# facebookresearch/robust_cvd

Measured on NVIDIA H100. Metric: flow_residual_constraints_per_sec_per_gn_iteration, higher is better.
Workload: dtype f64

## Files before the change

### robust_cvd_b200/csrc/rcvd_linalg.cuh

```cuda
#pragma once
#include "rcvd_device.cuh"

namespace rcvd {

constexpr int kPotrfThreads = 256;

__global__ void __launch_bounds__(kPotrfThreads) k_potrf_panel(double* __restrict__ Lb, double* __restrict__ invT,
                                                                const int* __restrict__ frames, int npad, int jb, int* __restrict__ fail) {
  __shared__ double D[16][17];
  __shared__ double Di[16][17];
  const int frame = frames[blockIdx.x];
  double* A = Lb + (size_t)frame * npad * npad;
  double* iT = invT + (size_t)frame * npad * 16;
  const int tid = threadIdx.x;
  const int j0 = jb * 16;
  {
    const int r = tid >> 4, cc = tid & 15;
    D[r][cc] = (cc <= r) ? A[(size_t)(j0 + r) * npad + j0 + cc] : 0.0;
  }
  __syncthreads();
  if (tid < 32) {
    const int i = tid;
    for (int j = 0; j < 16; ++j) {
      if (i == j) {
        double d = D[j][j];
        for (int q = 0; q < j; ++q) d -= D[j][q] * D[j][q];
        if (!(d > 0.0) || !isfinite(d)) { *fail = 1; d = 1.0; }
        D[j][j] = sqrt(d);
      }
      __syncwarp();
      if (i > j && i < 16) {
        double s = D[i][j];
        for (int q = 0; q < j; ++q) s -= D[i][q] * D[j][q];
        D[i][j] = s / D[j][j];
      }
      __syncwarp();
    }
    if (i < 16) {
      const int cidx = i;
      double xcol[16];
#pragma unroll
      for (int r = 0; r < 16; ++r) {
        double s = (r == cidx) ? 1.0 : 0.0;
#pragma unroll
        for (int q = 0; q < 16; ++q) if (q < r) s -= D[r][q] * xcol[q];
        xcol[r] = (r < cidx) ? 0.0 : s / D[r][r];
      }
#pragma unroll
      for (int r = 0; r < 16; ++r) Di[r][cidx] = xcol[r];
    }
  }
  __syncthreads();
  {
    const int r = tid >> 4, cc = tid & 15;
    A[(size_t)(j0 + r) * npad + j0 + cc] = D[r][cc];
    iT[(size_t)jb * 256 + r * 16 + cc] = Di[r][cc];
  }
  const int below = npad - (j0 + 16);
  for (int rr = tid; rr < below; rr += kPotrfThreads) {
    double a[16], xo[16];
    double* row = A + (size_t)(j0 + 16 + rr) * npad + j0;
#pragma unroll
    for (int q = 0; q < 16; ++q) a[q] = row[q];
#pragma unroll
    for (int cc = 0; cc < 16; ++cc) {
      double s = 0.0;
#pragma unroll
      for (int q = 0; q < 16; ++q) if (q <= cc) s += a[q] * Di[cc][q];
      xo[cc] = s;
    }
#pragma unroll
    for (int q = 0; q < 16; ++q) row[q] = xo[q];
  }
}

constexpr int kPotrfSmemThreads = 512;
constexpr int kTileSz = 256;
__host__ __device__ inline size_t potrf_smem_bytes(int npad) { const int nt = npad / 16; return (size_t)(nt * (nt + 1) / 2 + 1) * kTileSz * sizeof(double); }
__device__ __forceinline__ int swz(int r, int k) { return r * 16 + (k ^ ((r & 3) << 2)); }
__device__ __forceinline__ void cp_async16_fwd(void* smem, const void* gmem) {
  const unsigned sa = (unsigned)__cvta_generic_to_shared(smem);
  asm volatile("cp.async.cg.shared.global [%0], [%1], 16;" ::"r"(sa), "l"(gmem) : "memory");
}
__device__ __forceinline__ void dmma_8x8x4_fwd(double& c0, double& c1, double a, double b) {
  asm volatile("mma.sync.aligned.m8n8k4.row.col.f64.f64.f64.f64 {%0,%1}, {%2}, {%3}, {%0,%1};"
               : "+d"(c0), "+d"(c1) : "d"(a), "d"(b));
}

__device__ __forceinline__ void tile_mma_nt(const double* __restrict__ At, const double* __restrict__ Bt, double acc[2][2][2], int g, int t) {
#pragma unroll
  for (int k4 = 0; k4 < 4; ++k4) {
    double af[2], bf[2];
#pragma unroll
    for (int i = 0; i < 2; ++i) { af[i] = At[swz(i * 8 + g, k4 * 4 + t)]; bf[i] = Bt[swz(i * 8 + g, k4 * 4 + t)]; }
#pragma unroll
    for (int i = 0; i < 2; ++i)
#pragma unroll
      for (int j = 0; j < 2; ++j) dmma_8x8x4_fwd(acc[i][j][0], acc[i][j][1], af[i], bf[j]);
  }
}

__device__ __forceinline__ void warp_chol16(double* __restrict__ D, double* __restrict__ pinv, int lane, int* __restrict__ fail) {
  const int i = lane & 15;
  double a[16];
#pragma unroll
  for (int c = 0; c < 16; ++c) a[c] = (c <= i) ? D[swz(i, c)] : 0.0;
#pragma unroll
  for (int j = 0; j < 16; ++j) {
    double d = __shfl_sync(0xffffffffu, a[j], j);
    if (!(d > 0.0) || !isfinite(d)) { if (lane == 0) *fail = 1; d = 1.0; }
    const double pi = rsqrt(d);
    const double lij = (i == j) ? d * pi : a[j] * pi;
    if (i >= j) a[j] = lij;
    if (lane == 0) pinv[j] = pi;
#pragma unroll
    for (int c = 0; c < 16; ++c) {
      if (c > j) {
        const double lcj = __shfl_sync(0xffffffffu, a[j], c);
        if (i >= c) a[c] -= lij * lcj;
      }
    }
  }
  if (lane < 16) {
#pragma unroll
    for (int c = 0; c < 16; ++c) D[swz(i, c)] = a[c];
  }
}

#ifdef RCVD_POTRF_PHASES
__device__ long long g_potrf_phase[16];
#define POTRF_PHASE(n) do { if (threadIdx.x == 0 && blockIdx.x == 0) { const long long now_ = clock64(); g_potrf_phase[n] += now_ - last_; last_ = now_; } } while (0)
#define CHOL_PHASE(n) do { if (threadIdx.x == 0 && blockIdx.x == 0) { const long long now_ = clock64(); g_potrf_phase[n] += now_ - cl_; cl_ = now_; } } while (0)
#else
#define CHOL_PHASE(n) do { } while (0)
#define POTRF_PHASE(n) do { } while (0)
#endif

__device__ __forceinline__ void warp_chol16_blocked(double* __restrict__ D, double* __restrict__ pinv, int lane, int* __restrict__ fail) {
  const int g = lane >> 2, t = lane & 3;
  double c[3][2];
  const int ui[3] = {0, 1, 1}, uj[3] = {0, 0, 1};
#pragma unroll
  for (int u = 0; u < 3; ++u) { const double2 v = *reinterpret_cast<const double2*>(&D[swz(8 * ui[u] + g, 8 * uj[u] + 2 * t)]); c[u][0] = v.x; c[u][1] = v.y; }
  bool bad = false;
#ifdef RCVD_POTRF_PHASES
  long long cl_ = clock64();
#endif
#pragma unroll
  for (int b = 0; b < 4; ++b) {
    const int k0 = 4 * b;
    if (b > 0) {
#pragma unroll
      for (int u = 0; u < 3; ++u) if (8 * uj[u] + 2 * t >= k0) *reinterpret_cast<double2*>(&D[swz(8 * ui[u] + g, 8 * uj[u] + 2 * t)]) = make_double2(c[u][0], c[u][1]);
    }
    __syncwarp();
    double a00 = D[swz(k0, k0)], a10 = D[swz(k0 + 1, k0)], a11 = D[swz(k0 + 1, k0 + 1)], a20 = D[swz(k0 + 2, k0)], a21 = D[swz(k0 + 2, k0 + 1)],
           a22 = D[swz(k0 + 2, k0 + 2)], a30 = D[swz(k0 + 3, k0)], a31 = D[swz(k0 + 3, k0 + 1)], a32 = D[swz(k0 + 3, k0 + 2)], a33 = D[swz(k0 + 3, k0 + 3)];
    CHOL_PHASE(8);
    double t01 = a10 * a10;
    double det01 = fma(a00, a11, -t01);
    if (!(a00 > 0.0) || !isfinite(a00)) { bad = true; a00 = 1.0; det01 = 1.0; }
    if (!(det01 > 0.0) || !isfinite(det01)) { bad = true; det01 = a00; }
    const double p0 = rsqrt(a00), r01 = rsqrt(det01);
    const double sq0 = a00 * p0;
    const double p1 = r01 * sq0;
    const double l11 = det01 * r01 * p0;
    const double l10 = a10 * p0, l20 = a20 * p0, l30 = a30 * p0;
    const double l21 = (a21 - l20 * l10) * p1, l31 = (a31 - l30 * l10) * p1;
    double b22 = fma(-l21, l21, fma(-l20, l20, a22)), b33 = fma(-l31, l31, fma(-l30, l30, a33));
    const double b32 = fma(-l31, l21, fma(-l30, l20, a32));
    double det23 = fma(b22, b33, -(b32 * b32));
    if (!(b22 > 0.0) || !isfinite(b22)) { bad = true; b22 = 1.0; det23 = 1.0; }
    if (!(det23 > 0.0) || !isfinite(det23)) { bad = true; det23 = b22; }
    const double p2 = rsqrt(b22), r23 = rsqrt(det23);
    const double sq2 = b22 * p2;
    const double p3 = r23 * sq2;
    const double l33 = det23 * r23 * p2;
    const double l32 = b32 * p2;
    CHOL_PHASE(9);
    const int r = lane & 15;
    const bool below = lane < 16 && r >= k0 + 4;
    double x0 = D[swz(r, k0)] * p0;
    double x1 = (D[swz(r, k0 + 1)] - x0 * l10) * p1;
    double x2 = (D[swz(r, k0 + 2)] - x0 * l20 - x1 * l21) * p2;
    double x3 = (D[swz(r, k0 + 3)] - x0 * l30 - x1 * l31 - x2 * l32) * p3;
    if (below) { D[swz(r, k0)] = x0; D[swz(r, k0 + 1)] = x1; D[swz(r, k0 + 2)] = x2; D[swz(r, k0 + 3)] = x3; }
    __syncwarp();
    CHOL_PHASE(10);
    if (lane == 0) {
      *reinterpret_cast<double2*>(&D[swz(k0, k0)]) = make_double2(sq0, 0.0);         *reinterpret_cast<double2*>(&D[swz(k0, k0 + 2)]) = make_double2(0.0, 0.0);
      *reinterpret_cast<double2*>(&D[swz(k0 + 1, k0)]) = make_double2(l10, l11);     *reinterpret_cast<double2*>(&D[swz(k0 + 1, k0 + 2)]) = make_double2(0.0, 0.0);
      *reinterpret_cast<double2*>(&D[swz(k0 + 2, k0)]) = make_double2(l20, l21);          *reinterpret_cast<double2*>(&D[swz(k0 + 2, k0 + 2)]) = make_double2(sq2, 0.0);
      *reinterpret_cast<double2*>(&D[swz(k0 + 3, k0)]) = make_double2(l30, l31);          *reinterpret_cast<double2*>(&D[swz(k0 + 3, k0 + 2)]) = make_double2(l32, l33);
      *reinterpret_cast<double2*>(&pinv[k0]) = make_double2(p0, p1);                      *reinterpret_cast<double2*>(&pinv[k0 + 2]) = make_double2(p2, p3);
    }
    if (b < 3) {
      double pa[2];
#pragma unroll
      for (int i = 0; i < 2; ++i) { const int r = 8 * i + g; pa[i] = r >= k0 + 4 ? D[swz(r, k0 + t)] : 0.0; }
#pragma unroll
      for (int u = 0; u < 3; ++u) dmma_8x8x4_fwd(c[u][0], c[u][1], -pa[ui[u]], pa[uj[u]]);
    }
    CHOL_PHASE(11);
  }
  if (bad && lane == 0) *fail = 1;
}


__global__ void __launch_bounds__(kPotrfSmemThreads) k_potrf_smem(double* __restrict__ Lb, double* __restrict__ invT,
                                                                   const int* __restrict__ frames, int npad, int* __restrict__ fail, int chain_warp) {
  extern __shared__ __align__(16) double tiles[];
  const int frame = frames[blockIdx.x];
  double* A = Lb + (size_t)frame * npad * npad;
  double* iT = invT + (size_t)frame * npad * 16;
  const int nt = npad / 16, ntl = nt * (nt + 1) / 2;
  double* pinv = tiles + (size_t)ntl * kTileSz;
  const int tid = threadIdx.x, warp = tid >> 5, lane = tid & 31, nw = kPotrfSmemThreads / 32;
  const int g = lane >> 2, t = lane & 3;
#ifdef RCVD_POTRF_PHASES
  long long last_ = clock64();
#endif
  for (int idx = tid; idx < ntl * 128; idx += kPotrfSmemThreads) {
    const int tl = idx >> 7, e = idx & 127, r = e >> 3, c = (e & 7) * 2;
    int ti = (int)((sqrtf(8.f * tl + 1.f) - 1.f) * 0.5f);
    while ((ti + 1) * (ti + 2) / 2 <= tl) ++ti;
    while (ti * (ti + 1) / 2 > tl) --ti;
    const int tj = tl - ti * (ti + 1) / 2;
    cp_async16_fwd(&tiles[(size_t)tl * kTileSz + swz(r, c)], &A[(size_t)(ti * 16 + r) * npad + tj * 16 + c]);
  }
  asm volatile("cp.async.commit_group;" ::: "memory");
  asm volatile("cp.async.wait_group 0;" ::: "memory");
  __syncthreads();
  POTRF_PHASE(0);
  if (warp == 0) { if (chain_warp & 2) warp_chol16_blocked(tiles, pinv, lane, fail); else warp_chol16(tiles, pinv, lane, fail); }
  __syncthreads();
  POTRF_PHASE(1);
  for (int jb = 0; jb < nt; ++jb) {
    const double* D = tiles + (size_t)(jb * (jb + 1) / 2 + jb) * kTileSz;
    const double* pv = pinv + jb * 16;
    const int rows = (nt - jb - 1) * 16;
    const bool chain = (chain_warp & 1) != 0;
    int prow = -1;
    const int nwork = nw - 1, widx = warp - 1;
    if (chain) { if (warp == 0) { if (lane < 16 && rows > 0) prow = lane; } else if (widx * 32 + lane < rows - 16) prow = 16 + widx * 32 + lane; }
    else if (tid < rows) prow = tid;
    if (chain && warp != 0) asm volatile("bar.sync 2, %0;" ::"n"(kPotrfSmemThreads) : "memory");
    if (prow >= 0) {
      const int ti = jb + 1 + (prow >> 4), r = prow & 15;
      double* Tt = tiles + (size_t)(ti * (ti + 1) / 2 + jb) * kTileSz;
      double a[16];
#pragma unroll
      for (int q = 0; q < 16; q += 2) { const double2 v = *reinterpret_cast<const double2*>(&Tt[swz(r, q)]); a[q] = v.x; a[q + 1] = v.y; }
#pragma unroll
      for (int q = 0; q < 16; q += 2) {
        const double2 pq = *reinterpret_cast<const double2*>(&pv[q]);
        const double2 dq = *reinterpret_cast<const double2*>(&D[swz(q + 1, q)]);
        a[q] *= pq.x;
        a[q + 1] = (a[q + 1] - a[q] * dq.x) * pq.y;
#pragma unroll
        for (int c = 0; c < 16; ++c) if (c > q + 1) { const double2 l = *reinterpret_cast<const double2*>(&D[swz(c, q)]); a[c] -= a[q] * l.x; a[c] -= a[q + 1] * l.y; }
      }
#pragma unroll
      for (int q = 0; q < 16; q += 2) *reinterpret_cast<double2*>(&Tt[swz(r, q)]) = make_double2(a[q], a[q + 1]);
    } else if (warp == nw - 1 && lane < 16) {
      const int cidx = lane;
      double xcol[16];
#pragma unroll
      for (int r = 0; r < 16; ++r) xcol[r] = (r == cidx) ? 1.0 : 0.0;
#pragma unroll
      for (int q = 0; q < 16; q += 2) {
        const double2 pq = *reinterpret_cast<const double2*>(&pv[q]);
        const double2 dq = *reinterpret_cast<const double2*>(&D[swz(q + 1, q)]);
        xcol[q] *= pq.x;
        xcol[q + 1] = (xcol[q + 1] - xcol[q] * dq.x) * pq.y;
#pragma unroll
        for (int r = 0; r < 16; ++r) if (r > q + 1) { const double2 l = *reinterpret_cast<const double2*>(&D[swz(r, q)]); xcol[r] -= l.x * xcol[q]; xcol[r] -= l.y * xcol[q + 1]; }
      }
#pragma unroll
      for (int r = 0; r < 16; ++r) iT[(size_t)jb * 256 + r * 16 + cidx] = xcol[r];
    }
    POTRF_PHASE(2);
    if (!chain) __syncthreads();
    else if (warp != 0) asm volatile("bar.sync 3, %0;" ::"n"(kPotrfSmemThreads - 32) : "memory");
    POTRF_PHASE(3);
    const int m = nt - jb - 1, ntr = m * (m + 1) / 2;
    auto upd_tile = [&](int gi, int gj) -> double* {
      const double* Xi = tiles + (size_t)(gi * (gi + 1) / 2 + jb) * kTileSz;
      const double* Xj = tiles + (size_t)(gj * (gj + 1) / 2 + jb) * kTileSz;
      double* Ct = tiles + (size_t)(gi * (gi + 1) / 2 + gj) * kTileSz;
      double acc[2][2][2] = {{{0.0, 0.0}, {0.0, 0.0}}, {{0.0, 0.0}, {0.0, 0.0}}};
      tile_mma_nt(Xi, Xj, acc, g, t);
#pragma unroll
      for (int i = 0; i < 2; ++i)
#pragma unroll
        for (int j = 0; j < 2; ++j) {
          double2* ptr = reinterpret_cast<double2*>(&Ct[swz(i * 8 + g, j * 8 + 2 * t)]);
          double2 v = *ptr; v.x -= acc[i][j][0]; v.y -= acc[i][j][1]; *ptr = v;
        }
      return Ct;
    };
    auto tile_of = [&](int tl, int& gi, int& gj) {
      int ti = (int)((sqrtf(8.f * tl + 1.f) - 1.f) * 0.5f);
      while ((ti + 1) * (ti + 2) / 2 <= tl) ++ti;
      while (ti * (ti + 1) / 2 > tl) --ti;
      gi = jb + 1 + ti; gj = jb + 1 + (tl - ti * (ti + 1) / 2);
    };
    if (chain) {
      if (warp == 0) {
        double* Ct = nullptr;
        if (ntr > 0) { __syncwarp(); Ct = upd_tile(jb + 1, jb + 1); }
        __threadfence_block();
        asm volatile("bar.arrive 2, %0;" ::"n"(kPotrfSmemThreads) : "memory");
        POTRF_PHASE(4);
        if (ntr > 0) { __syncwarp(); if (chain_warp & 2) warp_chol16_blocked(Ct, pinv + (jb + 1) * 16, lane, fail); else warp_chol16(Ct, pinv + (jb + 1) * 16, lane, fail); }
        POTRF_PHASE(5);
      } else {
        for (int tl = 1 + widx; tl < ntr; tl += nwork) { int gi, gj; tile_of(tl, gi, gj); upd_tile(gi, gj); }
      }
    } else {
      for (int tl = warp; tl < ntr; tl += nw) {
        int gi, gj; tile_of(tl, gi, gj);
        double* Ct = upd_tile(gi, gj);
        if (tl == 0) { __syncwarp(); if (chain_warp & 2) warp_chol16_blocked(Ct, pinv + (jb + 1) * 16, lane, fail); else warp_chol16(Ct, pinv + (jb + 1) * 16, lane, fail); }
      }
    }
    POTRF_PHASE(6);
    __syncthreads();
    POTRF_PHASE(7);
  }
  for (int idx = tid; idx < ntl * 128; idx += kPotrfSmemThreads) {
    const int tl = idx >> 7, e = idx & 127, r = e >> 3, c = (e & 7) * 2;
    int ti = (int)((sqrtf(8.f * tl + 1.f) - 1.f) * 0.5f);
    while ((ti + 1) * (ti + 2) / 2 <= tl) ++ti;
    while (ti * (ti + 1) / 2 > tl) --ti;
    const int tj = tl - ti * (ti + 1) / 2;
    double2 v = *reinterpret_cast<const double2*>(&tiles[(size_t)tl * kTileSz + swz(r, c)]);
    if (ti == tj) { if (c > r) v.x = 0.0; if (c + 1 > r) v.y = 0.0; }
    *reinterpret_cast<double2*>(&A[(size_t)(ti * 16 + r) * npad + tj * 16 + c]) = v;
  }
}

__global__ void __launch_bounds__(256) k_trinv(const double* __restrict__ Lb, const double* __restrict__ invT, double* __restrict__ invL,
                                                const int* __restrict__ frames, int npad) {
  extern __shared__ double Z[];
  __shared__ double W[16][17];
  const int frame = frames[blockIdx.y];
  const int j = blockIdx.x;
  const int nt = npad / 16;
  double* Lrow_s = Z + (size_t)nt * 256;
  const int ldp = npad + 1;
  const double* A = Lb + (size_t)frame * npad * npad;
  const double* iT = invT + (size_t)frame * npad * 16;
  double* out = invL + (size_t)frame * npad * npad;
  const int tid = threadIdx.x, r = tid >> 4, c = tid & 15;
  for (int i = 0; i < j; ++i) out[(size_t)(i * 16 + r) * npad + j * 16 + c] = 0.0;
  Z[(size_t)j * 256 + tid] = iT[(size_t)j * 256 + tid];
  out[(size_t)(j * 16 + r) * npad + j * 16 + c] = Z[(size_t)j * 256 + tid];
  __syncthreads();
  for (int i = j + 1; i < nt; ++i) {
    const int kw = (i - j) * 16;
    for (int e = tid; e < 16 * kw; e += 256) { const int rr = e / kw, kk = e % kw; Lrow_s[rr * ldp + kk] = A[(size_t)(i * 16 + rr) * npad + j * 16 + kk]; }
    __syncthreads();
    double s0 = 0.0, s1 = 0.0, s2 = 0.0, s3 = 0.0;
    const double* lr = Lrow_s + r * ldp;
    const double* zp = Z + (size_t)j * 256 + c;
    for (int kk = 0; kk < kw; kk += 4) {
      s0 += lr[kk] * zp[(size_t)kk * 16]; s1 += lr[kk + 1] * zp[(size_t)(kk + 1) * 16];
      s2 += lr[kk + 2] * zp[(size_t)(kk + 2) * 16]; s3 += lr[kk + 3] * zp[(size_t)(kk + 3) * 16];
    }
    W[r][c] = (s0 + s1) + (s2 + s3);
    __syncthreads();
    double zv = 0.0;
    const double* ti = iT + (size_t)i * 256;
#pragma unroll
    for (int q = 0; q < 16; ++q) zv -= ti[r * 16 + q] * W[q][c];
    Z[(size_t)i * 256 + tid] = zv;
    out[(size_t)(i * 16 + r) * npad + j * 16 + c] = zv;
    __syncthreads();
  }
}

struct GemmTask { int dst; int first; int count; int lower_only; };

constexpr int kGemmLd = 20;

__device__ __forceinline__ void cp_async16(void* smem, const void* gmem, bool valid) {
  const unsigned s = (unsigned)__cvta_generic_to_shared(smem);
  const int sz = valid ? 16 : 0;
  asm volatile("cp.async.cg.shared.global [%0], [%1], 16, %2;" ::"r"(s), "l"(gmem), "r"(sz) : "memory");
}
__device__ __forceinline__ void cp_async_commit() { asm volatile("cp.async.commit_group;" ::: "memory"); }
template <int N> __device__ __forceinline__ void cp_async_wait() { asm volatile("cp.async.wait_group %0;" ::"n"(N) : "memory"); }

__device__ __forceinline__ void dmma_8x8x4(double& c0, double& c1, double a, double b) {
  asm volatile("mma.sync.aligned.m8n8k4.row.col.f64.f64.f64.f64 {%0,%1}, {%2}, {%3}, {%0,%1};"
               : "+d"(c0), "+d"(c1) : "d"(a), "d"(b));
}
__device__ __forceinline__ void dmma_16x8x4(double& c0, double& c1, double& c2, double& c3, double a0, double a1, double b) {
  asm volatile("mma.sync.aligned.m16n8k4.row.col.f64.f64.f64.f64 {%0,%1,%2,%3}, {%4,%5}, {%6}, {%0,%1,%2,%3};"
               : "+d"(c0), "+d"(c1), "+d"(c2), "+d"(c3) : "d"(a0), "d"(a1), "d"(b));
}

template <int NI, int NJ, int K4 = 4>
__device__ __forceinline__ void gemm_stage(const double* __restrict__ as, const double* __restrict__ bsm, double (&acc)[4][4][2], int wm, int wn, int g, int t) {
#pragma unroll
  for (int k4 = 0; k4 < K4; ++k4) {
    double af[NI > 0 ? NI : 1], bf[NJ > 0 ? NJ : 1];
#pragma unroll
    for (int i = 0; i < NI; ++i) af[i] = as[(wm + i * 8 + g) * kGemmLd + k4 * 4 + t];
#pragma unroll
    for (int j = 0; j < NJ; ++j) bf[j] = bsm[(wn + j * 8 + g) * kGemmLd + k4 * 4 + t];
#pragma unroll
    for (int i = 0; i < NI; ++i)
#pragma unroll
      for (int j = 0; j < NJ; ++j) dmma_8x8x4(acc[i][j][0], acc[i][j][1], af[i], bf[j]);
  }
}

__global__ void __launch_bounds__(128, 4) k_gemm_nt(double* __restrict__ dst, const double* __restrict__ Abase, const double* __restrict__ Bbase,
                                                  const GemmTask* __restrict__ tasks, const int2* __restrict__ pairs,
                                                  int npad, int neff, double alpha, double beta) {
  __shared__ __align__(16) double As[2][64 * kGemmLd];
  __shared__ __align__(16) double Bs[2][64 * kGemmLd];
  const GemmTask task = tasks[blockIdx.z];
  const int m0 = blockIdx.y * 64, n0 = blockIdx.x * 64;
  if ((task.lower_only & 1) && n0 > m0) return;
  const size_t bs = (size_t)npad * npad;
  const int tid = threadIdx.x, warp = tid >> 5, lane = tid & 31;
  const int wm = (warp >> 1) * 32, wn = (warp & 1) * 32;
  const int g = lane >> 2, t = lane & 3;
  const int kchunks = (task.lower_only & 2) ? min(npad, n0 + 64) / 16 : npad / 16;
  const int total = task.count * kchunks;
  const int ni = min(4, max(0, (neff - (m0 + wm)) / 8)), nj = min(4, max(0, (neff - (n0 + wn)) / 8));
  const int lastk = (task.lower_only & 2) ? -1 : kchunks - 1;
  const int tailk4 = (neff - 16 * (npad / 16 - 1) + 3) / 4;
  double acc[4][4][2];
#pragma unroll
  for (int i = 0; i < 4; ++i)
#pragma unroll
    for (int j = 0; j < 4; ++j) { acc[i][j][0] = 0.0; acc[i][j][1] = 0.0; }

  auto load_stage = [&](int st, int kk) {
    const int2 pr = pairs[task.first + kk / kchunks];
    const int k0 = (kk % kchunks) * 16;
    const double* Ag = Abase + (size_t)pr.x * bs + k0;
    const double* Bg = Bbase + (size_t)pr.y * bs + k0;
#pragma unroll
    for (int q = 0; q < 4; ++q) {
      const int cidx = tid + q * 128;
      const int row = cidx >> 3, kc = (cidx & 7) * 2;
      const bool va = (m0 + row) < npad, vb = (n0 + row) < npad;
      cp_async16(&As[st][row * kGemmLd + kc], Ag + (size_t)(va ? m0 + row : 0) * npad + kc, va);
      cp_async16(&Bs[st][row * kGemmLd + kc], Bg + (size_t)(vb ? n0 + row : 0) * npad + kc, vb);
    }
    cp_async_commit();
  };

  if (total > 0) load_stage(0, 0);
  for (int kk = 0; kk < total; ++kk) {
    const int st = kk & 1;
    if (kk + 1 < total) { load_stage(st ^ 1, kk + 1); cp_async_wait<1>(); } else { cp_async_wait<0>(); }
    __syncthreads();
    const double* as = As[st]; const double* bsm = Bs[st];
    const bool tail = (kk % kchunks) == lastk && tailk4 == 2;
#define RCVD_GS(NI_, NJ_) case NI_ * 8 + NJ_: if (tail) gemm_stage<NI_, NJ_, 2>(as, bsm, acc, wm, wn, g, t); else gemm_stage<NI_, NJ_, 4>(as, bsm, acc, wm, wn, g, t); break;
    if (ni == 4 && nj == 4 && !tail) gemm_stage<4, 4, 4>(as, bsm, acc, wm, wn, g, t);
    else switch (ni * 8 + nj) {
      RCVD_GS(4, 4) RCVD_GS(4, 3) RCVD_GS(4, 2) RCVD_GS(4, 1)
      RCVD_GS(3, 4) RCVD_GS(3, 3) RCVD_GS(3, 2) RCVD_GS(3, 1)
      RCVD_GS(2, 4) RCVD_GS(2, 3) RCVD_GS(2, 2) RCVD_GS(2, 1)
      RCVD_GS(1, 4) RCVD_GS(1, 3) RCVD_GS(1, 2) RCVD_GS(1, 1)
      default: break;
    }
#undef RCVD_GS
    __syncthreads();
  }
  double* C = dst + (size_t)task.dst * bs;
#pragma unroll
  for (int i = 0; i < 4; ++i) {
    const int row = m0 + wm + i * 8 + g;
    if (row >= neff) continue;
#pragma unroll
    for (int j = 0; j < 4; ++j) {
      const int col = n0 + wn + j * 8 + 2 * t;
      if (col >= neff) continue;
      double2* ptr = reinterpret_cast<double2*>(C + (size_t)row * npad + col);
      double2 o;
      if (beta != 0.0) { o = *ptr; o.x = beta * o.x + alpha * acc[i][j][0]; o.y = beta * o.y + alpha * acc[i][j][1]; }
      else { o.x = alpha * acc[i][j][0]; o.y = alpha * acc[i][j][1]; }
      *ptr = o;
    }
  }
}

__global__ void __launch_bounds__(128, 4) k_potrf_trail(double* __restrict__ Lb, const int* __restrict__ frames, int npad, int jb) {
  __shared__ __align__(16) double Ps[2][64 * kGemmLd];
  const int frame = frames[blockIdx.y];
  double* A = Lb + (size_t)frame * npad * npad;
  const int j0 = jb * 16, j1 = j0 + 16;
  int ti = (int)((sqrtf(8.f * blockIdx.x + 1.f) - 1.f) * 0.5f);
  while ((ti + 1) * (ti + 2) / 2 <= (int)blockIdx.x) ++ti;
  while (ti * (ti + 1) / 2 > (int)blockIdx.x) --ti;
  const int tj = blockIdx.x - ti * (ti + 1) / 2;
  const int m0 = j1 + ti * 64, n0 = j1 + tj * 64;
  const int tid = threadIdx.x, warp = tid >> 5, lane = tid & 31, g = lane >> 2, t = lane & 3;
  const int wm = (warp >> 1) * 32, wn = (warp & 1) * 32;
  for (int e = tid; e < 64 * 8; e += 128) {
    const int row = e >> 3, kc = (e & 7) * 2;
    const bool va = (m0 + row) < npad, vb = (n0 + row) < npad;
    cp_async16(&Ps[0][row * kGemmLd + kc], A + (size_t)(va ? m0 + row : 0) * npad + j0 + kc, va);
    cp_async16(&Ps[1][row * kGemmLd + kc], A + (size_t)(vb ? n0 + row : 0) * npad + j0 + kc, vb);
  }
  cp_async_commit(); cp_async_wait<0>();
  __syncthreads();
  const int ni = min(4, max(0, (npad - (m0 + wm)) / 8)), nj = min(4, max(0, (npad - (n0 + wn)) / 8));
  double acc[4][4][2];
#pragma unroll
  for (int i = 0; i < 4; ++i)
#pragma unroll
    for (int j = 0; j < 4; ++j) { acc[i][j][0] = 0.0; acc[i][j][1] = 0.0; }
  if (ni == 4 && nj == 4) gemm_stage<4, 4>(Ps[0], Ps[1], acc, wm, wn, g, t);
  else if (ni == 4 && nj == 2) gemm_stage<4, 2>(Ps[0], Ps[1], acc, wm, wn, g, t);
  else if (ni == 2 && nj == 4) gemm_stage<2, 4>(Ps[0], Ps[1], acc, wm, wn, g, t);
  else if (ni == 2 && nj == 2) gemm_stage<2, 2>(Ps[0], Ps[1], acc, wm, wn, g, t);
#pragma unroll
  for (int i = 0; i < 4; ++i) {
    const int row = m0 + wm + i * 8 + g;
    if (i >= ni) continue;
#pragma unroll
    for (int j = 0; j < 4; ++j) {
      const int col = n0 + wn + j * 8 + 2 * t;
      if (j >= nj || col > row) continue;
      double* ptr = A + (size_t)row * npad + col;
      if (col + 1 <= row) { double2 o = *reinterpret_cast<double2*>(ptr); o.x -= acc[i][j][0]; o.y -= acc[i][j][1]; *reinterpret_cast<double2*>(ptr) = o; }
      else ptr[0] -= acc[i][j][0];
    }
  }
}

struct TrsmTask { int dst; int src; int kframe; };
constexpr int kTrsmRW = 8;
constexpr int kTrsmStrip = 4 * kTrsmRW;
__host__ __device__ inline size_t trsm_ll_smem_bytes(int npad, int ahead = 2) { return ((size_t)kTrsmStrip * (npad + 4) + ahead * 16 * (size_t)(npad + 4) + ahead * 16 * 20) * sizeof(double); }

template <int kTrsmAhead>
__global__ void __launch_bounds__(128) k_trsm_ll(double* __restrict__ T, const double* __restrict__ Lb, const double* __restrict__ invT,
                                                  const TrsmTask* __restrict__ tasks, int npad) {
  extern __shared__ __align__(16) double smx[];
  const int ld = npad + 4;
  double* Xs = smx;
  double* Ls = smx + (size_t)kTrsmStrip * ld;
  double* Ds = Ls + (size_t)kTrsmAhead * 16 * ld;
  const TrsmTask task = tasks[blockIdx.y];
  const int m0 = blockIdx.x * kTrsmStrip;
  const size_t bs = (size_t)npad * npad;
  const double* A = Lb + (size_t)task.src * bs;
  const double* Lk = Lb + (size_t)task.kframe * bs;
  const double* iT = invT + (size_t)task.kframe * npad * 16;
  double* X = T + (size_t)task.dst * bs;
  const int tid = threadIdx.x, warp = tid >> 5, lane = tid & 31, g = lane >> 2, t = lane & 3;
  const int nt = npad / 16;
  const int rows = min(kTrsmStrip, npad - m0);
  for (int r = tid >> 3; r < kTrsmStrip; r += 16) {
    const bool v = r < rows;
    const double* src = A + (size_t)(v ? m0 + r : 0) * npad;
    for (int c = (tid & 7) * 2; c < npad; c += 16) cp_async16(&Xs[(size_t)r * ld + c], src + c, v);
  }
  auto stage = [&](int jt) {
    if (jt < nt) {
      double* ls = Ls + (size_t)(jt % kTrsmAhead) * 16 * ld; double* dsm = Ds + (jt % kTrsmAhead) * 320;
      const int kw = jt * 16;
      { const int r = tid >> 3; const double* src = Lk + (size_t)(jt * 16 + r) * npad; for (int c = (tid & 7) * 2; c < kw; c += 16) cp_async16(&ls[(size_t)r * ld + c], src + c, true); }
      { const int r = tid >> 3, c = (tid & 7) * 2; cp_async16(&dsm[r * 20 + c], iT + (size_t)jt * 256 + r * 16 + c, true); }
    }
    cp_async_commit();
  };
#pragma unroll
  for (int q = 0; q < kTrsmAhead; ++q) stage(q);
  constexpr int NI = kTrsmRW / 8;
  const int wr = warp * kTrsmRW;
  for (int jt = 0; jt < nt; ++jt) {
    cp_async_wait<kTrsmAhead - 1>();
    __syncthreads();
    const double* ls = Ls + (size_t)(jt % kTrsmAhead) * 16 * ld; const double* dsm = Ds + (jt % kTrsmAhead) * 320;
    double acc[NI][2][2];
#pragma unroll
    for (int i = 0; i < NI; ++i) { acc[i][0][0] = acc[i][0][1] = acc[i][1][0] = acc[i][1][1] = 0.0; }
    {
      double af[2][4][NI], bf[2][4][2];
      auto frag = [&](int kt, int buf) {
#pragma unroll
        for (int q = 0; q < 4; ++q) {
#pragma unroll
          for (int i = 0; i < NI; ++i) af[buf][q][i] = Xs[(size_t)(wr + i * 8 + g) * ld + kt * 16 + q * 4 + t];
#pragma unroll
          for (int j = 0; j < 2; ++j) bf[buf][q][j] = ls[(size_t)(j * 8 + g) * ld + kt * 16 + q * 4 + t];
        }
      };
      if (jt > 0) frag(0, 0);
      for (int kt = 0; kt < jt; kt += 2) {
        if (kt + 1 < jt) frag(kt + 1, 1);
#pragma unroll
        for (int q = 0; q < 4; ++q)
#pragma unroll
          for (int i = 0; i < NI; ++i)
#pragma unroll
            for (int j = 0; j < 2; ++j) dmma_8x8x4(acc[i][j][0], acc[i][j][1], af[0][q][i], bf[0][q][j]);
        if (kt + 1 < jt) {
          if (kt + 2 < jt) frag(kt + 2, 0);
#pragma unroll
          for (int q = 0; q < 4; ++q)
#pragma unroll
            for (int i = 0; i < NI; ++i)
#pragma unroll
              for (int j = 0; j < 2; ++j) dmma_8x8x4(acc[i][j][0], acc[i][j][1], af[1][q][i], bf[1][q][j]);
        }
      }
    }
#pragma unroll
    for (int i = 0; i < NI; ++i)
#pragma unroll
      for (int j = 0; j < 2; ++j) {
        double2* ptr = reinterpret_cast<double2*>(&Xs[(size_t)(wr + i * 8 + g) * ld + jt * 16 + j * 8 + 2 * t]);
        double2 v = *ptr; v.x -= acc[i][j][0]; v.y -= acc[i][j][1]; *ptr = v;
      }
    __syncwarp();
    double out[NI][2][2];
#pragma unroll
    for (int i = 0; i < NI; ++i) { out[i][0][0] = out[i][0][1] = out[i][1][0] = out[i][1][1] = 0.0; }
#pragma unroll
    for (int k4 = 0; k4 < 4; ++k4) {
      double af[NI], bf[2];
#pragma unroll
      for (int i = 0; i < NI; ++i) af[i] = Xs[(size_t)(wr + i * 8 + g) * ld + jt * 16 + k4 * 4 + t];
#pragma unroll
      for (int j = 0; j < 2; ++j) bf[j] = dsm[(j * 8 + g) * 20 + k4 * 4 + t];
#pragma unroll
      for (int i = 0; i < NI; ++i)
#pragma unroll
        for (int j = 0; j < 2; ++j) dmma_8x8x4(out[i][j][0], out[i][j][1], af[i], bf[j]);
    }
    __syncwarp();
#pragma unroll
    for (int i = 0; i < NI; ++i)
#pragma unroll
      for (int j = 0; j < 2; ++j) {
        const int r = wr + i * 8 + g, cidx = jt * 16 + j * 8 + 2 * t;
        const double2 v = make_double2(out[i][j][0], out[i][j][1]);
        *reinterpret_cast<double2*>(&Xs[(size_t)r * ld + cidx]) = v;
        if (r < rows) *reinterpret_cast<double2*>(&X[(size_t)(m0 + r) * npad + cidx]) = v;
      }
    __syncthreads();
    stage(jt + kTrsmAhead);
  }
}

__global__ void __launch_bounds__(256) k_fwd_diag_sub(const double* __restrict__ Lb, const double* __restrict__ invT, const double* __restrict__ rhs,
                                                       double* __restrict__ y, const int* __restrict__ frames, int npad) {
  extern __shared__ double vs[];
  double* tmp = vs + npad;
  const int frame = frames[blockIdx.x];
  const double* A = Lb + (size_t)frame * npad * npad; const double* iT = invT + (size_t)frame * npad * 16;
  const double* b = rhs + (size_t)frame * npad;
  const int tid = threadIdx.x, r = tid >> 4, c = tid & 15, nt = npad / 16;
  for (int jt = 0; jt < nt; ++jt) {
    double s = 0.0;
    const double* row = A + (size_t)(jt * 16 + r) * npad;
    for (int k = c; k < jt * 16; k += 16) s += row[k] * vs[k];
#pragma unroll
    for (int o = 8; o > 0; o >>= 1) s += __shfl_xor_sync(0xffffffffu, s, o);
    if (c == 0) tmp[r] = b[jt * 16 + r] - s;
    __syncthreads();
    if (tid < 16) {
      double acc = 0.0;
#pragma unroll
      for (int q = 0; q < 16; ++q) acc += iT[(size_t)jt * 256 + tid * 16 + q] * tmp[q];
      vs[jt * 16 + tid] = acc;
      y[(size_t)frame * npad + jt * 16 + tid] = acc;
    }
    __syncthreads();
  }
}
__global__ void __launch_bounds__(256) k_bwd_diag_sub(const double* __restrict__ Lb, const double* __restrict__ invT, const double* __restrict__ yin,
                                                       double* __restrict__ x, const int* __restrict__ frames, int npad) {
  extern __shared__ double vs[];
  double* tmp = vs + npad;
  const int frame = frames[blockIdx.x];
  const double* A = Lb + (size_t)frame * npad * npad; const double* iT = invT + (size_t)frame * npad * 16;
  const double* b = yin + (size_t)frame * npad;
  const int tid = threadIdx.x, r = tid >> 4, c = tid & 15, nt = npad / 16;
  for (int jt = nt - 1; jt >= 0; --jt) {
    double s = 0.0;
    for (int k = (jt + 1) * 16 + r; k < npad; k += 16) s += A[(size_t)k * npad + jt * 16 + c] * vs[k];
    __shared__ double red[256];
    red[tid] = s;
    __syncthreads();
    if (tid < 16) {
      double acc = 0.0;
#pragma unroll
      for (int q = 0; q < 16; ++q) acc += red[q * 16 + tid];
      tmp[tid] = b[jt * 16 + tid] - acc;
    }
    __syncthreads();
    if (tid < 16) {
      double acc = 0.0;
#pragma unroll
      for (int q = 0; q < 16; ++q) acc += iT[(size_t)jt * 256 + q * 16 + tid] * tmp[q];
      vs[jt * 16 + tid] = acc;
      x[(size_t)frame * npad + jt * 16 + tid] = acc;
    }
    __syncthreads();
  }
}

__global__ void __launch_bounds__(256) k_fwd_diag(const double* __restrict__ invL, const double* __restrict__ rhs, double* __restrict__ y,
                                                   const int* __restrict__ frames, int npad) {
  const int frame = frames[blockIdx.y];
  const int row = blockIdx.x * 8 + (threadIdx.x >> 5);
  const int lane = threadIdx.x & 31;
  if (row >= npad) return;
  const double* M = invL + (size_t)frame * npad * npad + (size_t)row * npad;
  const double* b = rhs + (size_t)frame * npad;
  double s = 0.0;
  for (int q = lane; q <= row; q += 32) s += M[q] * b[q];
  s = warp_sum(s);
  if (lane == 0) y[(size_t)frame * npad + row] = s;
}
struct SolveTask { int blk; int r; int k; };
__global__ void __launch_bounds__(256) k_fwd_update(const double* __restrict__ T, const double* __restrict__ y, double* __restrict__ rhs,
                                                     const SolveTask* __restrict__ tasks, int npad) {
  const SolveTask tk = tasks[blockIdx.y];
  const int row = blockIdx.x * 8 + (threadIdx.x >> 5);
  const int lane = threadIdx.x & 31;
  if (row >= npad) return;
  const double* M = T + (size_t)tk.blk * npad * npad + (size_t)row * npad;
  const double* v = y + (size_t)tk.k * npad;
  double s = 0.0;
  for (int q = lane; q < npad; q += 32) s += M[q] * v[q];
  s = warp_sum(s);
  if (lane == 0) red_add(rhs + (size_t)tk.r * npad + row, -s);
}
__global__ void __launch_bounds__(256) k_bwd_update(const double* __restrict__ T, const double* __restrict__ x, double* __restrict__ y,
                                                     const SolveTask* __restrict__ tasks, int npad) {
  __shared__ double red[8][33];
  const SolveTask tk = tasks[blockIdx.y];
  const int cl = threadIdx.x & 31, rg = threadIdx.x >> 5;
  const int j = blockIdx.x * 32 + cl;
  double acc = 0.0;
  if (j < npad) {
    const double* M = T + (size_t)tk.blk * npad * npad + j;
    const double* xr = x + (size_t)tk.r * npad;
    for (int i = rg; i < npad; i += 8) acc += M[(size_t)i * npad] * xr[i];
  }
  red[rg][cl] = acc;
  __syncthreads();
  if (rg == 0 && j < npad) {
    double s = 0.0;
#pragma unroll
    for (int q = 0; q < 8; ++q) s += red[q][cl];
    if (s != 0.0) red_add(y + (size_t)tk.k * npad + j, -s);
  }
}
__global__ void __launch_bounds__(256) k_bwd_diag(const double* __restrict__ invL, const double* __restrict__ y, double* __restrict__ x,
                                                   const int* __restrict__ frames, int npad) {
  __shared__ double red[8][33];
  const int frame = frames[blockIdx.y];
  const int cl = threadIdx.x & 31, rg = threadIdx.x >> 5;
  const int j = blockIdx.x * 32 + cl;
  double acc = 0.0;
  if (j < npad) {
    const double* M = invL + (size_t)frame * npad * npad + j;
    const double* v = y + (size_t)frame * npad;
    const int i0 = j - (j % 8) + rg;
    for (int i = (i0 < j ? i0 + 8 : i0); i < npad; i += 8) acc += M[(size_t)i * npad] * v[i];
  }
  red[rg][cl] = acc;
  __syncthreads();
  if (rg == 0 && j < npad) {
    double s = 0.0;
#pragma unroll
    for (int q = 0; q < 8; ++q) s += red[q][cl];
    x[(size_t)frame * npad + j] = s;
  }
}

constexpr int kSubChunk = 64;
constexpr int kSubThreads = 256;
struct SubTask { int type; int blk; int r; int k; int chunk; };
struct SubCounters { int* ticket; int* fin; int* fdone; int* bin; int* bdone; const int* fin_need; const int* bin_need; };

__device__ __forceinline__ int ld_acquire_gpu(const int* p) { int v; asm volatile("ld.acquire.gpu.global.s32 %0, [%1];" : "=r"(v) : "l"(p) : "memory"); return v; }
__device__ __forceinline__ void sub_wait(const int* c, int need) { while (ld_acquire_gpu(c) < need) __nanosleep(20); }

__device__ __forceinline__ void red_release_add(int* p, int v) { asm volatile("red.release.gpu.global.add.s32 [%0], %1;" ::"l"(p), "r"(v) : "memory"); }
__device__ __forceinline__ double2 ldcg2(const double* p) { return __ldcg(reinterpret_cast<const double2*>(p)); }

__global__ void __launch_bounds__(kSubThreads) k_substitution(const double* __restrict__ invL, const double* __restrict__ T, double* rhs, double* y, double* x,
                                                              const SubTask* __restrict__ tasks, int ntasks, SubCounters cn, int npad) {
  extern __shared__ __align__(16) double red[];
  __shared__ int s_task;
  const int tid = threadIdx.x, warp = tid >> 5, lane = tid & 31;
  const int nchunks = (npad + kSubChunk - 1) / kSubChunk;
  const size_t bs = (size_t)npad * npad;
  for (;;) {
    if (tid == 0) s_task = atomicAdd(cn.ticket, 1);
    __syncthreads();
    const int ti = s_task;
    if (ti >= ntasks) break;
    const SubTask tk = tasks[ti];
    const int c0 = tk.chunk * kSubChunk, c1 = min(npad, c0 + kSubChunk);
    const double* vin = tk.type == 0 ? rhs + (size_t)tk.k * npad : (tk.type == 2 ? x + (size_t)tk.r * npad : y + (size_t)tk.k * npad);
    const double* M = (tk.type == 0 || tk.type == 3) ? invL + (size_t)tk.k * bs : T + (size_t)tk.blk * bs;
    auto dep_wait = [&]() {
      if (tid == 0) {
        if (tk.type == 0) sub_wait(cn.fin + tk.k, cn.fin_need[tk.k]);
        else if (tk.type == 1) sub_wait(cn.fdone + tk.k, nchunks);
        else if (tk.type == 2) sub_wait(cn.bdone + tk.r, nchunks);
        else { sub_wait(cn.fdone + tk.k, nchunks); sub_wait(cn.bin + tk.k, cn.bin_need[tk.k]); }
      }
      __syncthreads();
    };
    if (tk.type <= 1) {
      constexpr int RW = kSubChunk / (kSubThreads / 32);
      const int r0 = c0 + warp * RW;
      double acc[RW];
#pragma unroll
      for (int i = 0; i < RW; ++i) acc[i] = 0.0;
      for (int qb = 0; qb < npad; qb += 256) {
        double2 m[4][RW];
#pragma unroll
        for (int qi = 0; qi < 4; ++qi) {
          const int q = qb + qi * 64 + 2 * lane;
#pragma unroll
          for (int i = 0; i < RW; ++i) {
            const int row = r0 + i;
            const int len = tk.type == 0 ? row + 1 : npad;
            m[qi][i] = (row < c1 && q < len) ? *reinterpret_cast<const double2*>(M + (size_t)row * npad + q) : make_double2(0.0, 0.0);
            if (q + 1 >= len) m[qi][i].y = 0.0;
          }
        }
        if (qb == 0) dep_wait();
        double2 v[4];
#pragma unroll
        for (int qi = 0; qi < 4; ++qi) { const int q = qb + qi * 64 + 2 * lane; v[qi] = q < npad ? ldcg2(vin + q) : make_double2(0.0, 0.0); }
#pragma unroll
        for (int qi = 0; qi < 4; ++qi)
#pragma unroll
          for (int i = 0; i < RW; ++i) acc[i] += m[qi][i].x * v[qi].x + m[qi][i].y * v[qi].y;
      }
#pragma unroll
      for (int i = 0; i < RW; ++i) {
        const double sum = warp_sum(acc[i]);
        const int row = r0 + i;
        if (lane == 0 && row < c1) { if (tk.type == 0) y[(size_t)tk.k * npad + row] = sum; else red_add(rhs + (size_t)tk.r * npad + row, -sum); }
      }
    } else {
      const int cl = tid & 31, rg = tid >> 5, j = c0 + 2 * cl;
      double ax = 0.0, ay = 0.0;
      const int ifirst = tk.type == 3 ? j + ((rg - j) & 7) : rg;
      for (int ib = ifirst; ib < npad || ib == ifirst; ib += 256) {
        double2 m[32];
#pragma unroll
        for (int u = 0; u < 32; ++u) { const int i = ib + 8 * u; m[u] = (i < npad && j < c1) ? *reinterpret_cast<const double2*>(M + (size_t)i * npad + j) : make_double2(0.0, 0.0); }
        if (ib == ifirst) dep_wait();
        double vi[32];
#pragma unroll
        for (int u = 0; u < 32; ++u) { const int i = ib + 8 * u; vi[u] = i < npad ? __ldcg(vin + i) : 0.0; }
#pragma unroll
        for (int u = 0; u < 32; ++u) { const int i = ib + 8 * u; ax += m[u].x * vi[u]; if (tk.type != 3 || i > j) ay += m[u].y * vi[u]; }
      }
      red[rg * (kSubChunk + 2) + 2 * cl] = ax; red[rg * (kSubChunk + 2) + 2 * cl + 1] = ay;
      __syncthreads();
      if (tid < kSubChunk && c0 + tid < c1) {
        double sum = 0.0;
#pragma unroll
        for (int q = 0; q < 8; ++q) sum += red[q * (kSubChunk + 2) + tid];
        if (tk.type == 3) x[(size_t)tk.k * npad + c0 + tid] = sum; else red_add(y + (size_t)tk.k * npad + c0 + tid, -sum);
      }
    }
    __syncthreads();
    if (tid == 0) red_release_add(tk.type == 0 ? cn.fdone + tk.k : (tk.type == 1 ? cn.fin + tk.r : (tk.type == 2 ? cn.bin + tk.k : cn.bdone + tk.k)), 1);
  }
}
__host__ __device__ inline size_t substitution_smem_bytes(int) { return (size_t)8 * (kSubChunk + 2) * sizeof(double); }

struct HBlock { int lblk; int r; int c; };
__global__ void __launch_bounds__(256) k_load_factor(const double* __restrict__ H, double* __restrict__ Lb, const HBlock* __restrict__ lb,
                                                      const double* __restrict__ S, const double* __restrict__ D2, int npad, int nf, const int* __restrict__ blist) {
  const int bid = blist ? blist[blockIdx.y] : blockIdx.y;
  const HBlock b = lb[bid];
  const int e = blockIdx.x * 256 + threadIdx.x;
  if (e >= npad * npad) return;
  const int i = e / npad, j = e % npad;
  const size_t bs = (size_t)npad * npad;
  double v = 0.0;
  if (b.r == b.c) {
    if (j > i) v = 0.0;
    else if (i >= nf) v = (i == j) ? 1.0 : 0.0;
    else {
      v = H[(size_t)b.lblk * bs + e] * S[(size_t)b.r * npad + i] * S[(size_t)b.c * npad + j];
      if (i == j) v += D2[(size_t)b.r * npad + i];
    }
  } else if (b.lblk >= 0 && i < nf && j < nf) {
    v = H[(size_t)b.lblk * bs + e] * S[(size_t)b.r * npad + i] * S[(size_t)b.c * npad + j];
  }
  Lb[(size_t)bid * bs + e] = v;
}

__global__ void __launch_bounds__(256) k_spmv_sym(const double* __restrict__ H, const HBlock* __restrict__ hb, const double* __restrict__ v,
                                                   double* __restrict__ out, int npad, const int* __restrict__ blist) {
  const int bid = blist ? blist[blockIdx.y] : blockIdx.y;
  const HBlock b = hb[bid];
  const int row = blockIdx.x * 8 + (threadIdx.x >> 5);
  const int lane = threadIdx.x & 31;
  if (row >= npad) return;
  const double* M = H + (size_t)bid * npad * npad + (size_t)row * npad;
  const double* vc = v + (size_t)b.c * npad;
  const double vr = v[(size_t)b.r * npad + row];
  double s = 0.0;
  if (b.r == b.c) {
    for (int q = lane; q <= row; q += 32) {
      const double m = M[q];
      s += m * vc[q];
      if (q < row && m != 0.0) red_add(out + (size_t)b.c * npad + q, m * vr);
    }
  } else {
    for (int q = lane; q < npad; q += 32) {
      const double m = M[q];
      s += m * vc[q];
      if (m != 0.0 && vr != 0.0) red_add(out + (size_t)b.c * npad + q, m * vr);
    }
  }
  s = warp_sum(s);
  if (lane == 0 && s != 0.0) red_add(out + (size_t)b.r * npad + row, s);
}

}
```

Before: 73.76 million.

## Use m16n8k4 DMMA in potrf, GEMM, and TRSM with transposed accumulation

Replaces pairs of m8n8k4 FP64 MMA instructions with single m16n8k4 instructions in the tile MMA, the in-warp Cholesky update, and the GEMM stage. The GEMM k-loop is now only partially unrolled. The TRSM kernel computes the transposed product (L as the A operand, X as the B operand) and splits the accumulation into four partial sums to shorten the dependency chain. It then writes results back transposed, using a swizzle and a shuffle to form coalesced double2 global stores. The aim is fewer MMA issues and more instruction-level parallelism, at the cost of more registers, scalar shared-memory scatter stores, and possible bank conflicts.

```diff
diff --git a/robust_cvd_b200/csrc/rcvd_linalg.cuh b/robust_cvd_b200/csrc/rcvd_linalg.cuh
--- a/robust_cvd_b200/csrc/rcvd_linalg.cuh
+++ b/robust_cvd_b200/csrc/rcvd_linalg.cuh
@@ -82,10 +82,14 @@
   const unsigned sa = (unsigned)__cvta_generic_to_shared(smem);
   asm volatile("cp.async.cg.shared.global [%0], [%1], 16;" ::"r"(sa), "l"(gmem) : "memory");
 }
-__device__ __forceinline__ void dmma_8x8x4_fwd(double& c0, double& c1, double a, double b) {
+__device__ __forceinline__ void dmma_8x8x4(double& c0, double& c1, double a, double b) {
   asm volatile("mma.sync.aligned.m8n8k4.row.col.f64.f64.f64.f64 {%0,%1}, {%2}, {%3}, {%0,%1};"
                : "+d"(c0), "+d"(c1) : "d"(a), "d"(b));
 }
+__device__ __forceinline__ void dmma_16x8x4(double& c0, double& c1, double& c2, double& c3, double a0, double a1, double b) {
+  asm volatile("mma.sync.aligned.m16n8k4.row.col.f64.f64.f64.f64 {%0,%1,%2,%3}, {%4,%5}, {%6}, {%0,%1,%2,%3};"
+               : "+d"(c0), "+d"(c1), "+d"(c2), "+d"(c3) : "d"(a0), "d"(a1), "d"(b));
+}
 
 __device__ __forceinline__ void tile_mma_nt(const double* __restrict__ At, const double* __restrict__ Bt, double acc[2][2][2], int g, int t) {
 #pragma unroll
@@ -94,9 +98,7 @@
 #pragma unroll
     for (int i = 0; i < 2; ++i) { af[i] = At[swz(i * 8 + g, k4 * 4 + t)]; bf[i] = Bt[swz(i * 8 + g, k4 * 4 + t)]; }
 #pragma unroll
-    for (int i = 0; i < 2; ++i)
-#pragma unroll
-      for (int j = 0; j < 2; ++j) dmma_8x8x4_fwd(acc[i][j][0], acc[i][j][1], af[i], bf[j]);
+    for (int j = 0; j < 2; ++j) dmma_16x8x4(acc[0][j][0], acc[0][j][1], acc[1][j][0], acc[1][j][1], af[0], af[1], bf[j]);
   }
 }
 
@@ -198,8 +200,8 @@
       double pa[2];
 #pragma unroll
       for (int i = 0; i < 2; ++i) { const int r = 8 * i + g; pa[i] = r >= k0 + 4 ? D[swz(r, k0 + t)] : 0.0; }
-#pragma unroll
-      for (int u = 0; u < 3; ++u) dmma_8x8x4_fwd(c[u][0], c[u][1], -pa[ui[u]], pa[uj[u]]);
+      dmma_16x8x4(c[0][0], c[0][1], c[1][0], c[1][1], -pa[0], -pa[1], pa[0]);
+      dmma_8x8x4(c[2][0], c[2][1], -pa[1], pa[1]);
     }
     CHOL_PHASE(11);
   }
@@ -392,18 +394,9 @@
 __device__ __forceinline__ void cp_async_commit() { asm volatile("cp.async.commit_group;" ::: "memory"); }
 template <int N> __device__ __forceinline__ void cp_async_wait() { asm volatile("cp.async.wait_group %0;" ::"n"(N) : "memory"); }
 
-__device__ __forceinline__ void dmma_8x8x4(double& c0, double& c1, double a, double b) {
-  asm volatile("mma.sync.aligned.m8n8k4.row.col.f64.f64.f64.f64 {%0,%1}, {%2}, {%3}, {%0,%1};"
-               : "+d"(c0), "+d"(c1) : "d"(a), "d"(b));
-}
-__device__ __forceinline__ void dmma_16x8x4(double& c0, double& c1, double& c2, double& c3, double a0, double a1, double b) {
-  asm volatile("mma.sync.aligned.m16n8k4.row.col.f64.f64.f64.f64 {%0,%1,%2,%3}, {%4,%5}, {%6}, {%0,%1,%2,%3};"
-               : "+d"(c0), "+d"(c1), "+d"(c2), "+d"(c3) : "d"(a0), "d"(a1), "d"(b));
-}
-
 template <int NI, int NJ, int K4 = 4>
 __device__ __forceinline__ void gemm_stage(const double* __restrict__ as, const double* __restrict__ bsm, double (&acc)[4][4][2], int wm, int wn, int g, int t) {
-#pragma unroll
+#pragma unroll 2
   for (int k4 = 0; k4 < K4; ++k4) {
     double af[NI > 0 ? NI : 1], bf[NJ > 0 ? NJ : 1];
 #pragma unroll
@@ -411,9 +404,13 @@
 #pragma unroll
     for (int j = 0; j < NJ; ++j) bf[j] = bsm[(wn + j * 8 + g) * kGemmLd + k4 * 4 + t];
 #pragma unroll
-    for (int i = 0; i < NI; ++i)
-#pragma unroll
-      for (int j = 0; j < NJ; ++j) dmma_8x8x4(acc[i][j][0], acc[i][j][1], af[i], bf[j]);
+    for (int i = 0; i + 1 < NI; i += 2)
+#pragma unroll
+      for (int j = 0; j < NJ; ++j) dmma_16x8x4(acc[i][j][0], acc[i][j][1], acc[i + 1][j][0], acc[i + 1][j][1], af[i], af[i + 1], bf[j]);
+    if (NI & 1) {
+#pragma unroll
+      for (int j = 0; j < NJ; ++j) dmma_8x8x4(acc[NI - 1][j][0], acc[NI - 1][j][1], af[NI - 1], bf[j]);
+    }
   }
 }
 
@@ -579,22 +576,25 @@
   for (int q = 0; q < kTrsmAhead; ++q) stage(q);
   constexpr int NI = kTrsmRW / 8;
   const int wr = warp * kTrsmRW;
+  const int esw = t >> 1;
   for (int jt = 0; jt < nt; ++jt) {
     cp_async_wait<kTrsmAhead - 1>();
     __syncthreads();
     const double* ls = Ls + (size_t)(jt % kTrsmAhead) * 16 * ld; const double* dsm = Ds + (jt % kTrsmAhead) * 320;
-    double acc[NI][2][2];
-#pragma unroll
-    for (int i = 0; i < NI; ++i) { acc[i][0][0] = acc[i][0][1] = acc[i][1][0] = acc[i][1][1] = 0.0; }
+    double part[4][NI][4];
+#pragma unroll
+    for (int q = 0; q < 4; ++q)
+#pragma unroll
+      for (int i = 0; i < NI; ++i) { part[q][i][0] = part[q][i][1] = part[q][i][2] = part[q][i][3] = 0.0; }
     {
-      double af[2][4][NI], bf[2][4][2];
+      double lf[2][4][2], xf[2][4][NI];
       auto frag = [&](int kt, int buf) {
 #pragma unroll
         for (int q = 0; q < 4; ++q) {
 #pragma unroll
-          for (int i = 0; i < NI; ++i) af[buf][q][i] = Xs[(size_t)(wr + i * 8 + g) * ld + kt * 16 + q * 4 + t];
-#pragma unroll
-          for (int j = 0; j < 2; ++j) bf[buf][q][j] = ls[(size_t)(j * 8 + g) * ld + kt * 16 + q * 4 + t];
+          for (int j = 0; j < 2; ++j) lf[buf][q][j] = ls[(size_t)(j * 8 + g) * ld + kt * 16 + q * 4 + t];
+#pragma unroll
+          for (int i = 0; i < NI; ++i) xf[buf][q][i] = Xs[(size_t)(wr + i * 8 + g) * ld + kt * 16 + q * 4 + t];
         }
       };
       if (jt > 0) frag(0, 0);
@@ -603,52 +603,60 @@
 #pragma unroll
         for (int q = 0; q < 4; ++q)
 #pragma unroll
-          for (int i = 0; i < NI; ++i)
-#pragma unroll
-            for (int j = 0; j < 2; ++j) dmma_8x8x4(acc[i][j][0], acc[i][j][1], af[0][q][i], bf[0][q][j]);
+          for (int i = 0; i < NI; ++i) dmma_16x8x4(part[q][i][0], part[q][i][1], part[q][i][2], part[q][i][3], lf[0][q][0], lf[0][q][1], xf[0][q][i]);
         if (kt + 1 < jt) {
           if (kt + 2 < jt) frag(kt + 2, 0);
 #pragma unroll
           for (int q = 0; q < 4; ++q)
 #pragma unroll
-            for (int i = 0; i < NI; ++i)
-#pragma unroll
-              for (int j = 0; j < 2; ++j) dmma_8x8x4(acc[i][j][0], acc[i][j][1], af[1][q][i], bf[1][q][j]);
+            for (int i = 0; i < NI; ++i) dmma_16x8x4(part[q][i][0], part[q][i][1], part[q][i][2], part[q][i][3], lf[1][q][0], lf[1][q][1], xf[1][q][i]);
         }
       }
     }
+    double acc[NI][4];
 #pragma unroll
     for (int i = 0; i < NI; ++i)
 #pragma unroll
-      for (int j = 0; j < 2; ++j) {
-        double2* ptr = reinterpret_cast<double2*>(&Xs[(size_t)(wr + i * 8 + g) * ld + jt * 16 + j * 8 + 2 * t]);
-        double2 v = *ptr; v.x -= acc[i][j][0]; v.y -= acc[i][j][1]; *ptr = v;
-      }
+      for (int m = 0; m < 4; ++m) acc[i][m] = (part[0][i][m] + part[1][i][m]) + (part[2][i][m] + part[3][i][m]);
+#pragma unroll
+    for (int i = 0; i < NI; ++i)
+#pragma unroll
+      for (int h = 0; h < 2; ++h)
+#pragma unroll
+        for (int e = 0; e < 2; ++e) {
+          const int es = e ^ esw;
+          double* ptr = &Xs[(size_t)(wr + i * 8 + 2 * t + es) * ld + jt * 16 + h * 8 + g];
+          *ptr -= es ? acc[i][2 * h + 1] : acc[i][2 * h];
+        }
     __syncwarp();
-    double out[NI][2][2];
-#pragma unroll
-    for (int i = 0; i < NI; ++i) { out[i][0][0] = out[i][0][1] = out[i][1][0] = out[i][1][1] = 0.0; }
+    double out[NI][4];
+#pragma unroll
+    for (int i = 0; i < NI; ++i) { out[i][0] = out[i][1] = out[i][2] = out[i][3] = 0.0; }
 #pragma unroll
     for (int k4 = 0; k4 < 4; ++k4) {
-      double af[NI], bf[2];
-#pragma unroll
-      for (int i = 0; i < NI; ++i) af[i] = Xs[(size_t)(wr + i * 8 + g) * ld + jt * 16 + k4 * 4 + t];
-#pragma unroll
-      for (int j = 0; j < 2; ++j) bf[j] = dsm[(j * 8 + g) * 20 + k4 * 4 + t];
-#pragma unroll
-      for (int i = 0; i < NI; ++i)
-#pragma unroll
-        for (int j = 0; j < 2; ++j) dmma_8x8x4(out[i][j][0], out[i][j][1], af[i], bf[j]);
+      double df[2], xf[NI];
+#pragma unroll
+      for (int j = 0; j < 2; ++j) df[j] = dsm[(j * 8 + g) * 20 + k4 * 4 + t];
+#pragma unroll
+      for (int i = 0; i < NI; ++i) xf[i] = Xs[(size_t)(wr + i * 8 + g) * ld + jt * 16 + k4 * 4 + t];
+#pragma unroll
+      for (int i = 0; i < NI; ++i) dmma_16x8x4(out[i][0], out[i][1], out[i][2], out[i][3], df[0], df[1], xf[i]);
     }
     __syncwarp();
+    const bool odd = g & 1;
 #pragma unroll
     for (int i = 0; i < NI; ++i)
 #pragma unroll
-      for (int j = 0; j < 2; ++j) {
-        const int r = wr + i * 8 + g, cidx = jt * 16 + j * 8 + 2 * t;
-        const double2 v = make_double2(out[i][j][0], out[i][j][1]);
-        *reinterpret_cast<double2*>(&Xs[(size_t)r * ld + cidx]) = v;
-        if (r < rows) *reinterpret_cast<double2*>(&X[(size_t)(m0 + r) * npad + cidx]) = v;
+      for (int h = 0; h < 2; ++h) {
+#pragma unroll
+        for (int e = 0; e < 2; ++e) {
+          const int es = e ^ esw;
+          Xs[(size_t)(wr + i * 8 + 2 * t + es) * ld + jt * 16 + h * 8 + g] = es ? out[i][2 * h + 1] : out[i][2 * h];
+        }
+        const double keep = odd ? out[i][2 * h + 1] : out[i][2 * h];
+        const double other = __shfl_xor_sync(0xffffffffu, odd ? out[i][2 * h] : out[i][2 * h + 1], 4);
+        const int r = wr + i * 8 + 2 * t + (odd ? 1 : 0), cidx = jt * 16 + h * 8 + (g & ~1);
+        if (r < rows) *reinterpret_cast<double2*>(&X[(size_t)(m0 + r) * npad + cidx]) = odd ? make_double2(other, keep) : make_double2(keep, other);
       }
     __syncthreads();
     stage(jt + kTrsmAhead);
```

Result: faster. 74.96 million, median of 6 (+1.6%).
